# Napoliee/Expressive-FastSpeech2-Mandarin

Hardware: AMD Instinct MI355X
Metric: mel-frames/sec/GPU (batch-64 synth) at 1/2/4/8 MI355X; RTF (higher is better)
Workload: dtype bf16; 1 GPU; cfg2: batch=64 x 64 phonemes per GPU, ESD-Chinese-Singing-MFA model.yaml, FastSpeech2.forward eval bf16; global_batch=64, seq_len=64, mel_frames_per_gpu_batch=24883, T_max=430, parallelism=dp1 (independent shards, no collective), hip_graph=True

## Files before the change

### expressive-fastspeech2-mandarin_amd/csrc/ffn.hip

```cpp
#include <cstdlib>
#include <type_traits>
#include <utility>

#include "conv_common.h"
#include "fs2_common.h"

namespace {

#ifndef FFN_TRACE
#define FFN_TRACE 0
#endif
#ifndef FFN_ABLATE
#define FFN_ABLATE 0
#endif

constexpr int kD = 256;
constexpr int kChunk = 256;
constexpr int kUnit = 4096;
constexpr int kDepth = 4;

struct FfnArgs {
  ConvArgs e;
  const bf16 *w;
  const float *b1;
  uint32_t w_bytes;
  int nsplit;
  int ntiles;
  int *cnt;
  void *part;
  int acquire;
  int out_sc1;
  int prefetch;
  uint32_t part_bytes;
  const bf16 *wq;
  const float *bq;
  bf16 *qkv;
  int64_t qs;
  uint32_t wq_bytes;
  int nq;
  const bf16 *att;
  int64_t as;
  uint32_t att_bytes;
  const bf16 *wfc;
  const float *bfc, *g1, *be1;
  float eps1;
};

constexpr int part_bytes(int MB) { return 4 * 4 * MB * 64 * 16; }

constexpr int64_t ffn_weight_elems(int KS, int F) { return (int64_t)F * KS * kD + (int64_t)kD * F; }

__device__ __forceinline__ int xchunk(int r, int c) { return c ^ ((r & 3) << 1) ^ ((r & 4) ? 9 : 0); }

template <int N, typename Fn, int... I>
__device__ __forceinline__ void static_for_impl(Fn &&f, std::integer_sequence<int, I...>) {
  (f(std::integral_constant<int, I>{}), ...);
}
template <int N, typename Fn>
__device__ __forceinline__ void static_for(Fn &&f) {
  static_for_impl<N>(f, std::make_integer_sequence<int, N>{});
}

constexpr int kLgkm0 = 0xC07F;
constexpr int vm_imm(int n) { return (n & 15) | ((n >> 4) << 14) | 0x0F70; }

template <bool FUSED>
__device__ __forceinline__ float sumsq4(const f32x4 &d) {
#pragma clang fp contract(off)
  if constexpr (FUSED)
    return __builtin_fmaf(d[0], d[0], d[1] * d[1]) + __builtin_fmaf(d[2], d[2], d[3] * d[3]);
  else
    return (d[0] * d[0] + d[1] * d[1]) + (d[2] * d[2] + d[3] * d[3]);
}

template <int KS, int NCH, int MB, bool PRE = false, int NW = 4>
__global__ __launch_bounds__(NW * 64, NW / 4) void ffn_fused_kernel(FfnArgs p) {
  static_assert(NW == 4 || (NW == 8 && PRE && MB == 7 && KS == 9 && NCH == 4),
                "eight waves: the packed unsplit 112-row PRE launch only");
  constexpr int JB = 16 / NW;
  constexpr int NT = NW * 64;
  constexpr int BM = 16 * MB;
  constexpr uint32_t kPartBytes = (uint32_t)part_bytes(MB);
  constexpr int XROWS = BM + KS - 1;
  constexpr int XPITCH = 544;
  constexpr int XPIECES = (XROWS * XPITCH + 1023) / 1024;
  constexpr int XP_PER_WAVE = (XPIECES + NW - 1) / NW;
  constexpr int ZERO_OFF = 0;
  constexpr int X_OFF = 512;
  constexpr int H_OFF = X_OFF + NW * XP_PER_WAVE * 1024;
  constexpr int F = NCH * kChunk;
  constexpr int B1_OFF = H_OFF + BM * 512;
  constexpr int EP_OFF = B1_OFF + F * 4;
  constexpr int RED_OFF = EP_OFF + 3 * kD * 4;
  constexpr int ATT_OFF = H_OFF;
  constexpr int RED0_OFF = ATT_OFF + NW * XP_PER_WAVE * 1024;
  constexpr int SMEM0 = RED_OFF + BM * 16;
  constexpr int VEC0_OFF = RED0_OFF + 64 * 16;
  constexpr int SMEM1 = PRE && VEC0_OFF + 3 * kD * 4 > SMEM0 ? VEC0_OFF + 3 * kD * 4 : SMEM0;
  constexpr int XCH_OFF = SMEM1;
  constexpr int SMEM = SMEM1 + (NW == 8 ? 4 * 8 * 64 * 4 : 0);
  static_assert(SMEM <= 163840, "LDS");
  static_assert(MB <= 8, "pair-exchange slots");
  static_assert(BM * 528 <= NW * XP_PER_WAVE * 1024, "Q|K|V staging fits in the x region");
  constexpr int NK1 = KS * (kD / 32);
  constexpr int NK2 = kChunk / 32;
  constexpr int DEPTH = kDepth;
  static_assert(NK1 % DEPTH == 0 && NK2 % DEPTH == 0, "static register-ring slots");
  constexpr int SCR_OFF = SMEM + (FFN_TRACE ? 256 : 0);
  __shared__ __attribute__((aligned(16))) char smem[SCR_OFF + (PRE ? 0 : 4096)];

  const ConvArgs &a = p.e;
  const uint64_t t_entry = FFN_TRACE ? __builtin_readcyclecounter() : 0;
  const int tid = threadIdx.x, lane = tid & 63;
  const int wv = __builtin_amdgcn_readfirstlane(tid >> 6);
  const int w = NW == 8 ? wv >> 1 : wv;
  const int hf = NW == 8 ? wv & 1 : 0;
  const int col0 = wv * (16 * JB);
  const int M = a.rows_dev != nullptr ? min(*a.rows_dev, a.M) : a.M;
  const int S = p.nsplit;
  int tile = blockIdx.x, split = 0;
  if (S > 1) {
    const int ntiles = p.ntiles;
    const int L = (blockIdx.x & 7) * (gridDim.x >> 3) + (blockIdx.x >> 3);
    split = L / ntiles;
    tile = L - split * ntiles;
    if (split >= S) return;
  }
  const int m0 = tile * BM;
  if (m0 >= M) return;
  const int nchunks = NCH / S, c0 = split * nchunks, cend = c0 + nchunks;
  const int pad = a.pad, T = a.T;

  int vmask[MB];
  int padmask = 0;
  int2 rq[MB];
  int64_t rl[MB];
  if (NW == 8 || a.row_pos != nullptr) {
#pragma unroll
    for (int mb = 0; mb < MB; ++mb) rq[mb] = a.row_pos[min(m0 + mb * 16 + (lane & 15), M - 1)];
  } else {
#pragma unroll
    for (int mb = 0; mb < MB; ++mb) {
      const int m = min(m0 + mb * 16 + (lane & 15), M - 1);
      rq[mb] = make_int2(m % T, T);
    }
    if (a.lens != nullptr) {
#pragma unroll
      for (int mb = 0; mb < MB; ++mb) rl[mb] = a.lens[min(m0 + mb * 16 + (lane & 15), M - 1) / T];
    } else {
#pragma unroll
      for (int mb = 0; mb < MB; ++mb) rl[mb] = T;
    }
  }
#pragma unroll
  for (int mb = 0; mb < MB; ++mb) {
    const int m = m0 + mb * 16 + (lane & 15);
    int tpos = 0, tlen = 0;
    if (m < M) {
      tpos = rq[mb].x;
      tlen = rq[mb].y;
      if (NW == 4 && a.row_pos == nullptr && (int64_t)tpos >= rl[mb]) padmask |= 1 << mb;
    }
    int v = 0;
#pragma unroll
    for (int tap = 0; tap < KS; ++tap) v |= ((unsigned)(tpos + tap - pad) < (unsigned)tlen ? 1 : 0) << tap;
    vmask[mb] = v;
  }
  auto vec_dma = [&](const float *src, int piece, char *dst) {
    __builtin_amdgcn_raw_ptr_buffer_load_lds(make_rsrc(src, (uint32_t)(piece + 1) * 1024u),
                                             (__attribute__((address_space(3))) void *)dst, 16,
                                             (uint32_t)piece * 1024u + (uint32_t)lane * 16u, 0, 0, 0);
  };
  auto load_vectors = [&]() {
    for (int pc = wv; pc < F / 256; pc += NW) vec_dma(p.b1, pc, smem + B1_OFF + pc * 1024);
    if (wv < 3) vec_dma(wv == 0 ? a.bias : wv == 1 ? a.gamma : a.beta, 0, smem + EP_OFF + wv * 1024);
  };
  if constexpr (!PRE) load_vectors();
  if (tid < 32) *reinterpret_cast<float4 *>(smem + ZERO_OFF + 16 * tid) = make_float4(0.f, 0.f, 0.f, 0.f);
#pragma unroll
  for (int mb = 0; mb < MB; ++mb) asm volatile("" ::"v"(vmask[mb]));

  auto stamp = [&](int i) {
    if (FFN_TRACE) {
      __builtin_amdgcn_sched_barrier(0);
      const uint64_t t = __builtin_readcyclecounter();
      if (tid == 0) *reinterpret_cast<uint64_t *>(smem + SMEM + 8 * i) = t;
      __builtin_amdgcn_sched_barrier(0);
    }
  };
  auto pair_sum = [&](auto &pv, const auto &sv) {
    if constexpr (NW == 8) {
      constexpr int N = sizeof(pv) / sizeof(float);
      float *xp = reinterpret_cast<float *>(smem + XCH_OFF) + w * 512 + lane;
      if (hf == 0) {
#pragma unroll
        for (int i = 0; i < N; ++i) xp[i * 64] = pv[i];
      }
      __builtin_amdgcn_s_waitcnt(kLgkm0);
      __builtin_amdgcn_sched_barrier(0);
      __builtin_amdgcn_s_barrier();
      __builtin_amdgcn_sched_barrier(0);
      if (hf == 1) {
#pragma unroll
        for (int i = 0; i < N; ++i) pv[i] = (xp[i * 64] + sv[0][i]) + sv[1][i];
      }
    }
  };
  const rsrc_t wr = make_rsrc(p.w, p.w_bytes);
  auto tile_dma_range = [&](const void *src, uint32_t bytes, int64_t stride, int off, int i0, int i1) {
    const rsrc_t sr = make_rsrc(src, bytes);
    const uint32_t srow = (uint32_t)stride * 2u;
#pragma unroll
    for (int i = i0; i < i1; ++i) {
      const int pc = wv + NW * i;
      const int o = pc * 1024 + lane * 16;
      const int r = o / XPITCH, within = o - r * XPITCH;
      const int gm = m0 - pad + r;
      const bool ok = r < XROWS && within < 512 && gm >= 0 && gm < M;
      __builtin_amdgcn_raw_ptr_buffer_load_lds(
          sr, (__attribute__((address_space(3))) void *)(smem + off + pc * 1024), 16,
          ok ? (uint32_t)gm * srow + (uint32_t)within : kOOB, 0, 0, 0);
    }
  };
  auto tile_dma = [&](const void *src, uint32_t bytes, int64_t stride, int off) {
    tile_dma_range(src, bytes, stride, off, 0, XP_PER_WAVE);
  };
  constexpr uint32_t W2_BASE = (uint32_t)(F * KS * kD * 2);
  const uint32_t lane_off = (uint32_t)lane * 16u + (uint32_t)hf * 2048u;
  auto base1 = [&](int c) { return (uint32_t)((c * 4 + w) * NK1) * (uint32_t)kUnit; };
  auto base2 = [&](int c) { return W2_BASE + (uint32_t)(w * (F / 32) + c * NK2) * (uint32_t)kUnit; };
  bf16x8 pa[DEPTH][JB];
  auto load_at = [&](auto S, uint32_t so) {
    constexpr int s = decltype(S)::value;
    if (FFN_ABLATE & 2) return;
    __builtin_amdgcn_sched_barrier(0);
#pragma unroll
    for (int jb = 0; jb < JB; ++jb) {
      auto v = __builtin_amdgcn_raw_buffer_load_b128(wr, lane_off + jb * 1024, (FFN_ABLATE & 8) ? 0u : so, 0);
      pa[s][jb] = __builtin_bit_cast(bf16x8, v);
    }
    __builtin_amdgcn_sched_barrier(0);
  };
  auto ring_start = [&]() {
    static_for<DEPTH>([&](auto I) { load_at(I, base1(c0) + (uint32_t)(decltype(I)::value * kUnit)); });
  };
  if constexpr (!PRE) {
    if (S > 1 && p.prefetch) {
      const int nch = cend - c0;
      const int p1 = nch * 4 * NK1 * 4, p2q = nch * NK2 * 4;
      const uint32_t g1 = (uint32_t)(c0 * 4 * NK1) * (uint32_t)kUnit;
      constexpr uint32_t W2B = (uint32_t)(F * KS * kD * 2);
      const int per_xcd = (int)(gridDim.x >> 3);
      const int me = (int)(blockIdx.x >> 3) * 4 + w, nw = per_xcd * 4;
      for (int i = 0, pc = me; i < 16 && pc < p1 + 4 * p2q; ++i, pc += nw) {
        uint32_t off;
        if (pc < p1) {
          off = g1 + (uint32_t)pc * 1024u;
        } else {
          const int j = pc - p1, ww = j / p2q, r = j - ww * p2q;
          off = W2B + (uint32_t)(ww * (F / 32) + c0 * NK2) * (uint32_t)kUnit + (uint32_t)r * 1024u;
        }
        __builtin_amdgcn_raw_ptr_buffer_load_lds(wr, (__attribute__((address_space(3))) void *)(smem + SCR_OFF + w * 1024),
                                                 16, off + (uint32_t)lane * 16u, 0, 0, 0);
      }
    }
    tile_dma(a.x, a.x_bytes, a.xs, X_OFF);
    ring_start();
  } else {
    const int hr = lane & 15, hq = lane >> 4;
    if (wv < 3) vec_dma(wv == 0 ? p.bfc : wv == 1 ? p.g1 : p.be1, 0, smem + VEC0_OFF + wv * 1024);
    const rsrc_t fr = make_rsrc(p.wfc, (uint32_t)(kD * kD * 2));
    const uint32_t lane_o = lane_off;
    bf16x8 wf[8][JB];
#pragma unroll
    for (int ks = 0; ks < 8; ++ks)
#pragma unroll
      for (int jb = 0; jb < JB; ++jb)
        wf[ks][jb] = __builtin_bit_cast(bf16x8, __builtin_amdgcn_raw_buffer_load_b128(
                                                    fr, lane_o + (uint32_t)(jb * 1024), (uint32_t)((w * 8 + ks) * kUnit), 0));
    constexpr int PRE_SPLIT = (64 * XPITCH + 1023) / 1024 / NW + 1;
    static_assert(NW * PRE_SPLIT * 1024 >= 64 * XPITCH && PRE_SPLIT <= XP_PER_WAVE, "row pass 0 pieces");
    tile_dma_range(p.att, p.att_bytes, p.as, ATT_OFF, 0, PRE_SPLIT);
    tile_dma_range(a.x, a.x_bytes, a.xs, X_OFF, 0, PRE_SPLIT);
    tile_dma_range(p.att, p.att_bytes, p.as, ATT_OFF, PRE_SPLIT, XP_PER_WAVE);
    tile_dma_range(a.x, a.x_bytes, a.xs, X_OFF, PRE_SPLIT, XP_PER_WAVE);
    stamp(21);
    __builtin_amdgcn_s_waitcnt(vm_imm(2 * (XP_PER_WAVE - PRE_SPLIT)));
    __builtin_amdgcn_s_waitcnt(kLgkm0);
    __builtin_amdgcn_s_barrier();
    stamp(22);
    float *red0 = reinterpret_cast<float *>(smem + RED0_OFF);
    static_for<(XROWS + 63) / 64>([&](auto PS) {
      constexpr int ps = decltype(PS)::value;
      if constexpr (ps == 1) {
        asm volatile("s_waitcnt vmcnt(0)" ::: "memory");
        __builtin_amdgcn_s_barrier();
      }
      f32x4 a0[JB][4];
#pragma unroll
      for (int jb = 0; jb < JB; ++jb)
#pragma unroll
        for (int mb = 0; mb < 4; ++mb) a0[jb][mb] = f32x4{0.f, 0.f, 0.f, 0.f};
#pragma unroll
      for (int ks = 0; ks < 8; ++ks) {
        bf16x8 fb[4];
#pragma unroll
        for (int mb = 0; mb < 4; ++mb) {
          const int r = min(64 * ps + 16 * mb + hr, XROWS - 1);
          fb[mb] = *reinterpret_cast<const bf16x8 *>(smem + ATT_OFF + r * XPITCH + ks * 64 + hq * 16);
        }
#pragma unroll
        for (int mb = 0; mb < 4; ++mb)
#pragma unroll
          for (int jb = 0; jb < JB; ++jb)
            a0[jb][mb] = __builtin_amdgcn_mfma_f32_16x16x32_bf16(wf[ks][jb], fb[mb], a0[jb][mb], 0, 0, 0);
      }
      float part[4] = {0.f, 0.f, 0.f, 0.f}, mean[4], var[4];
      float sv[JB][4];
#pragma unroll
      for (int jb = 0; jb < JB; ++jb) {
        const int n = (NW == 8 ? col0 : w * 64) + jb * 16 + 4 * hq;
        const float4 bb = *reinterpret_cast<const float4 *>(smem + VEC0_OFF + 4 * n);
#pragma unroll
        for (int mb = 0; mb < 4; ++mb) {
          const int r = 64 * ps + 16 * mb + hr, gm = m0 - pad + r;
          const bool ok = r < XROWS && gm >= 0 && gm < M;
          bf16x4 xv = {(bf16)0.f, (bf16)0.f, (bf16)0.f, (bf16)0.f};
          if (ok) xv = *reinterpret_cast<const bf16x4 *>(smem + X_OFF + r * XPITCH + n * 2);
          f32x4 v = a0[jb][mb];
          v[0] = v[0] + bb.x + (float)xv[0];
          v[1] = v[1] + bb.y + (float)xv[1];
          v[2] = v[2] + bb.z + (float)xv[2];
          v[3] = v[3] + bb.w + (float)xv[3];
          a0[jb][mb] = v;
          if constexpr (NW == 8) {
            sv[jb][mb] = (v[0] + v[1]) + (v[2] + v[3]);
            part[mb] += sv[jb][mb];
          } else {
            part[mb] += (v[0] + v[1]) + (v[2] + v[3]);
          }
        }
      }
      auto reduce4 = [&](float (&pv)[4], float (&tot)[4]) {
        pair_sum(pv, sv);
        float t[4];
#pragma unroll
        for (int mb = 0; mb < 4; ++mb) t[mb] = __shfl_xor(pv[mb], 16, 64);
#pragma unroll
        for (int mb = 0; mb < 4; ++mb) pv[mb] += t[mb];
#pragma unroll
        for (int mb = 0; mb < 4; ++mb) t[mb] = __shfl_xor(pv[mb], 32, 64);
        if (NW == 4 || hf == 1) {
#pragma unroll
          for (int mb = 0; mb < 4; ++mb) red0[(mb * 16 + hr) * 4 + w] = pv[mb] + t[mb];
        }
        __builtin_amdgcn_s_waitcnt(kLgkm0);
        __builtin_amdgcn_s_barrier();
#pragma unroll
        for (int mb = 0; mb < 4; ++mb) {
          const float4 r4 = *reinterpret_cast<const float4 *>(red0 + (mb * 16 + hr) * 4);
          tot[mb] = (r4.x + r4.y) + (r4.z + r4.w);
        }
        __builtin_amdgcn_s_waitcnt(kLgkm0);
        __builtin_amdgcn_s_barrier();
      };
      reduce4(part, mean);
#pragma unroll
      for (int mb = 0; mb < 4; ++mb) {
        mean[mb] *= 1.0f / kD;
        float ss = 0.f;
#pragma unroll
        for (int jb = 0; jb < JB; ++jb) {
          f32x4 d = a0[jb][mb];
          d[0] -= mean[mb];
          d[1] -= mean[mb];
          d[2] -= mean[mb];
          d[3] -= mean[mb];
          a0[jb][mb] = d;
          if constexpr (NW == 8) {
            if constexpr (ps == 0)
              sv[jb][mb] = sumsq4<true>(d);
            else if (jb == 0 && mb < 3 && hf == 0)
              sv[jb][mb] = sumsq4<true>(d);
            else
              sv[jb][mb] = sumsq4<false>(d);
            ss += sv[jb][mb];
          } else {
            ss += (d[0] * d[0] + d[1] * d[1]) + (d[2] * d[2] + d[3] * d[3]);
          }
        }
        part[mb] = ss;
      }
      reduce4(part, var);
      float rstd[4], keep[4] = {1.f, 1.f, 1.f, 1.f};
#pragma unroll
      for (int mb = 0; mb < 4; ++mb) rstd[mb] = 1.0f / sqrtf(var[mb] * (1.0f / kD) + p.eps1);
      if (NW == 4 && a.lens != nullptr) {
#pragma unroll
        for (int mb = 0; mb < 4; ++mb) {
          const int gm = m0 - pad + 64 * ps + 16 * mb + hr;
          if (gm >= 0 && gm < M) {
            const int bb = gm / T;
            keep[mb] = (int64_t)(gm - bb * T) < a.lens[bb] ? 1.0f : 0.0f;
          }
        }
      }
#pragma unroll
      for (int jb = 0; jb < JB; ++jb) {
        const int n = (NW == 8 ? col0 : w * 64) + jb * 16 + 4 * hq;
        const float4 g = *reinterpret_cast<const float4 *>(smem + VEC0_OFF + 4 * (kD + n));
        const float4 be = *reinterpret_cast<const float4 *>(smem + VEC0_OFF + 4 * (2 * kD + n));
#pragma unroll
        for (int mb = 0; mb < 4; ++mb) {
          const int r = 64 * ps + 16 * mb + hr;
          const f32x4 d = a0[jb][mb];
          bf16x4 o;
          o[0] = (bf16)((d[0] * rstd[mb] * g.x + be.x) * keep[mb]);
          o[1] = (bf16)((d[1] * rstd[mb] * g.y + be.y) * keep[mb]);
          o[2] = (bf16)((d[2] * rstd[mb] * g.z + be.z) * keep[mb]);
          o[3] = (bf16)((d[3] * rstd[mb] * g.w + be.w) * keep[mb]);
          if (r < XROWS) *reinterpret_cast<bf16x4 *>(smem + X_OFF + r * XPITCH + n * 2) = o;
        }
      }
      stamp(23 + ps);
    });
    __builtin_amdgcn_s_waitcnt(kLgkm0);
    __builtin_amdgcn_s_barrier();
    load_vectors();
    ring_start();
  }


  const int hrow0 = lane & 15;
  const int hi = lane >> 4;
  bf16x8 f0[MB], f1[MB];
  auto bases_x = [&](int tap, int (&ad)[MB]) {
    const int base = X_OFF + (hrow0 + tap) * XPITCH + hi * 16;
#pragma unroll
    for (int mb = 0; mb < MB; ++mb) {
      const int keep = (FFN_ABLATE & 16) ? -1 : __builtin_amdgcn_sbfe(vmask[mb], tap, 1);
      ad[mb] = (base + mb * 16 * XPITCH) & keep;
    }
  };
  auto issue_x = [&](const int (&ad)[MB], auto KSI, bf16x8 (&f)[MB]) {
    if (FFN_ABLATE & 4) return;
    constexpr int off = decltype(KSI)::value * 64;
#pragma unroll
    for (int mb = 0; mb < MB; ++mb) f[mb] = *reinterpret_cast<const bf16x8 *>(smem + ad[mb] + off);
  };
  auto read_h = [&](int q, bf16x8 (&f)[MB]) {
    if (FFN_ABLATE & 4) return;
    const char *hp = smem + H_OFF + hrow0 * 512 + (xchunk(hrow0, 4 * q + hi) << 4);
#pragma unroll
    for (int mb = 0; mb < MB; ++mb) f[mb] = *reinterpret_cast<const bf16x8 *>(hp + mb * 8192);
  };

  f32x4 acc1[JB][MB], acc2[JB][MB];
#pragma unroll
  for (int i = 0; i < JB; ++i)
#pragma unroll
    for (int j = 0; j < MB; ++j) {
      acc1[i][j] = f32x4{0.f, 0.f, 0.f, 0.f};
      acc2[i][j] = f32x4{0.f, 0.f, 0.f, 0.f};
    }
  auto mma = [&](f32x4 (&acc)[JB][MB], const bf16x8 (&fa)[JB], const bf16x8 (&fb)[MB]) {
    if (FFN_ABLATE & 1) return;
#pragma unroll
    for (int mb = 0; mb < MB; ++mb)
#pragma unroll
      for (int jb = 0; jb < JB; ++jb)
        acc[jb][mb] = __builtin_amdgcn_mfma_f32_16x16x32_bf16(fa[jb], fb[mb], acc[jb][mb], 0, 0, 0);
  };
  auto bar = []() {
    __builtin_amdgcn_sched_barrier(0);
    __builtin_amdgcn_s_barrier();
    __builtin_amdgcn_sched_barrier(0);
  };
  auto trace_dump = [&](int last) {
    if (FFN_TRACE) {
      uint64_t *o = S > 1 ? reinterpret_cast<uint64_t *>(static_cast<char *>(p.part) + p.part_bytes + 256u * blockIdx.x)
                          : reinterpret_cast<uint64_t *>(static_cast<char *>(a.out) + (size_t)(a.M - 1 - blockIdx.x) * a.os * 2);
      for (int i = 0; i < 25; ++i) o[i] = *reinterpret_cast<const uint64_t *>(smem + SMEM + 8 * i);
      o[28] = t_entry;
      o[29] = (uint64_t)split;
      o[30] = (uint64_t)last;
      o[31] = (uint64_t)25;
    }
  };
  stamp(0);

  auto write_h = [&](int c) {
    float z;
    asm volatile("v_mov_b32 %0, 0" : "=v"(z));
#pragma unroll
    for (int jb = 0; jb < JB; ++jb) {
      const int j = (NW == 8 ? col0 : w * 64) + jb * 16 + 4 * hi;
      const float4 bb = *reinterpret_cast<const float4 *>(smem + B1_OFF + 4 * (c * kChunk + j));
#pragma unroll
      for (int mb = 0; mb < MB; ++mb) {
        const f32x4 v = acc1[jb][mb];
        bf16x4 o;
        o[0] = (bf16)fmaxf(v[0] + bb.x, 0.f);
        o[1] = (bf16)fmaxf(v[1] + bb.y, 0.f);
        o[2] = (bf16)fmaxf(v[2] + bb.z, 0.f);
        o[3] = (bf16)fmaxf(v[3] + bb.w, 0.f);
        const int m = hrow0 + mb * 16;
        *reinterpret_cast<bf16x4 *>(smem + H_OFF + m * 512 + (xchunk(m, j >> 3) << 4) + (j & 7) * 2) = o;
        acc1[jb][mb] = f32x4{z, z, z, z};
      }
    }
  };

  asm volatile("s_waitcnt vmcnt(%0)" ::"n"(JB * DEPTH) : "memory");
  __builtin_amdgcn_s_waitcnt(kLgkm0);
  bar();
  stamp(1);
  int bxc[MB], bxn[MB];
  bases_x(0, bxc);
  issue_x(bxc, std::integral_constant<int, 0>{}, f0);

  static_assert(DEPTH == 4 && kD / 32 == 8, "8 units per tap, 4-unit ring");
  auto unit1 = [&](auto KSI, int c, int tap) {
    constexpr int ks = decltype(KSI)::value, s = ks % DEPTH;
    if constexpr (ks + 1 < 8) {
      if constexpr (ks & 1)
        issue_x(bxc, std::integral_constant<int, ks + 1>{}, f0);
      else
        issue_x(bxc, std::integral_constant<int, ks + 1>{}, f1);
    } else {
      issue_x(bxn, std::integral_constant<int, 0>{}, f0);
    }
    if constexpr (ks & 1)
      mma(acc1, pa[s], f1);
    else
      mma(acc1, pa[s], f0);
    const uint32_t k1 = (uint32_t)(tap * 8 + ks + DEPTH) * (uint32_t)kUnit;
    if constexpr (ks + DEPTH < 8) {
      load_at(std::integral_constant<int, s>{}, base1(c) + k1);
    } else {
      const bool more = tap + 1 < KS;
      load_at(std::integral_constant<int, s>{},
              more ? base1(c) + k1 : base2(c) + (uint32_t)(((2 * w + ks - DEPTH) & (NK2 - 1)) * kUnit));
    }
  };
#pragma nounroll
  for (int c = c0; c < cend; ++c) {
#pragma nounroll
    for (int tap = 0; tap < KS; ++tap) {
      bases_x(tap + 1, bxn);
      static_for<8>([&](auto KSI) { unit1(KSI, c, tap); });
#pragma unroll
      for (int mb = 0; mb < MB; ++mb) bxc[mb] = bxn[mb];
    }
    stamp(2 + 2 * (c - c0));
    bar();
    write_h(c);
    __builtin_amdgcn_s_waitcnt(kLgkm0);
    stamp(3 + 2 * (c - c0));
    if constexpr (NW == 8) bar();
    read_h(2 * w, f0);
    const uint32_t next1 = c + 1 < cend ? base1(c + 1) : 0u;
    static_for<NK2>([&](auto Q) {
      constexpr int q = decltype(Q)::value;
      constexpr int s = q % DEPTH;
      if constexpr (q == 1 && NW == 4) {
        __builtin_amdgcn_s_waitcnt(kLgkm0);
        bar();
      }
      const int qn = (2 * w + q + 1) & (NK2 - 1);
      if constexpr (q + 1 == NK2) {
        bases_x(0, bxc);
        issue_x(bxc, std::integral_constant<int, 0>{}, f0);
      }
      else if constexpr (q & 1)
        read_h(qn, f0);
      else
        read_h(qn, f1);
      if constexpr (q & 1)
        mma(acc2, pa[s], f1);
      else
        mma(acc2, pa[s], f0);
      if constexpr (q + DEPTH < NK2)
        load_at(std::integral_constant<int, s>{}, base2(c) + (uint32_t)(((2 * w + q + DEPTH) & (NK2 - 1)) * kUnit));
      else
        load_at(std::integral_constant<int, s>{}, next1 + (uint32_t)((q + DEPTH - NK2) * kUnit));
    });
  }

  stamp(2 + 2 * NCH);
  asm volatile("s_waitcnt vmcnt(0)" ::: "memory");
  __builtin_amdgcn_s_waitcnt(kLgkm0);
  stamp(4 + 2 * NCH);
  if constexpr (NW == 4) {
    if (S > 1) {
      const rsrc_t pr = make_rsrc(p.part, p.part_bytes);
      auto pofs = [&](int sp, int nb, int mb) {
        return (uint32_t)(tile * S + sp) * (uint32_t)kPartBytes + (uint32_t)((((w * 4 + nb) * MB + mb) * 64 + lane) * 16);
      };
#pragma unroll
      for (int nb = 0; nb < 4; ++nb)
#pragma unroll
        for (int mb = 0; mb < MB; ++mb)
          __builtin_amdgcn_raw_buffer_store_b128(__builtin_bit_cast(__attribute__((ext_vector_type(4))) unsigned, acc2[nb][mb]),
                                                 pr, pofs(split, nb, mb), 0, 16);
      asm volatile("s_waitcnt vmcnt(0)" ::: "memory");
      __syncthreads();
      int *flag = reinterpret_cast<int *>(smem + RED_OFF);
      if (tid == 0) {
        const int old = __hip_atomic_fetch_add(p.cnt + tile, 1, __ATOMIC_RELAXED, __HIP_MEMORY_SCOPE_AGENT);
        const int last = old == S - 1;
        if (last) {
          __hip_atomic_store(p.cnt + tile, 0, __ATOMIC_RELAXED, __HIP_MEMORY_SCOPE_AGENT);
          if (p.acquire) __builtin_amdgcn_fence(__ATOMIC_ACQUIRE, "agent");
        }
        *flag = last;
      }
      asm volatile("s_waitcnt vmcnt(0)" ::: "memory");
      __syncthreads();
      stamp(19);
      if (FFN_TRACE && !*flag) {
        if (tid == 0) trace_dump(0);
      }
      if (!*flag) return;
      __syncthreads();
#pragma unroll
      for (int nb = 0; nb < 4; ++nb)
#pragma unroll
        for (int mb = 0; mb < MB; ++mb) acc1[nb][mb] = f32x4{0.f, 0.f, 0.f, 0.f};
      if constexpr (MB <= 4) {
        f32x4 v[3][4][MB];
        static_for<3>([&](auto J) {
          constexpr int j = decltype(J)::value;
          if (j < S - 1) {
            const int sp = j + (j >= split ? 1 : 0);
#pragma unroll
            for (int nb = 0; nb < 4; ++nb)
#pragma unroll
              for (int mb = 0; mb < MB; ++mb)
                v[j][nb][mb] = __builtin_bit_cast(f32x4, __builtin_amdgcn_raw_buffer_load_b128(pr, pofs(sp, nb, mb), 0, 16));
          }
        });
        static_for<4>([&](auto SP) {
          constexpr int sp = decltype(SP)::value;
          constexpr int jlo = sp < 3 ? sp : 2, jhi = sp > 0 ? sp - 1 : 0;
          if (sp < S) {
#pragma unroll
            for (int nb = 0; nb < 4; ++nb)
#pragma unroll
              for (int mb = 0; mb < MB; ++mb)
                acc1[nb][mb] += sp < split ? v[jlo][nb][mb] : (sp == split ? acc2[nb][mb] : v[jhi][nb][mb]);
          }
        });
      } else {
        for (int sp = 0; sp < S; ++sp) {
          if (sp == split) {
#pragma unroll
            for (int nb = 0; nb < 4; ++nb)
#pragma unroll
              for (int mb = 0; mb < MB; ++mb) acc1[nb][mb] += acc2[nb][mb];
          } else {
            f32x4 v[4][MB];
#pragma unroll
            for (int nb = 0; nb < 4; ++nb)
#pragma unroll
              for (int mb = 0; mb < MB; ++mb)
                v[nb][mb] = __builtin_bit_cast(f32x4, __builtin_amdgcn_raw_buffer_load_b128(pr, pofs(sp, nb, mb), 0, 16));
#pragma unroll
            for (int nb = 0; nb < 4; ++nb)
#pragma unroll
              for (int mb = 0; mb < MB; ++mb) acc1[nb][mb] += v[nb][mb];
          }
        }
      }
#pragma unroll
      for (int nb = 0; nb < 4; ++nb)
#pragma unroll
        for (int mb = 0; mb < MB; ++mb) acc2[nb][mb] = acc1[nb][mb];
      stamp(20);
    }
  }
  {
    int lane_e = lane;
    if constexpr (NW == 8) asm volatile("" : "+v"(lane_e));
    const int hrow0 = lane_e & 15, hi = lane_e >> 4;
    float *red = reinterpret_cast<float *>(smem + RED_OFF);
    const float inv_n = 1.0f / 256.0f;
    float4 b2v[JB], gv[JB], bev[JB];
#pragma unroll
    for (int nb = 0; nb < JB; ++nb) {
      const int n = (NW == 8 ? col0 : w * 64) + nb * 16 + 4 * hi;
      b2v[nb] = *reinterpret_cast<const float4 *>(smem + EP_OFF + 4 * n);
      gv[nb] = *reinterpret_cast<const float4 *>(smem + EP_OFF + 4 * (kD + n));
      bev[nb] = *reinterpret_cast<const float4 *>(smem + EP_OFF + 4 * (2 * kD + n));
    }
    float part[MB];
    float sv[JB][MB];
#pragma unroll
    for (int mb = 0; mb < MB; ++mb) {
      const int xr = mb * 16 + hrow0 + pad;
      float sum = 0.f;
#pragma unroll
      for (int nb = 0; nb < JB; ++nb) {
        const int n = (NW == 8 ? col0 : w * 64) + nb * 16 + 4 * hi;
        const bf16x4 xv = *reinterpret_cast<const bf16x4 *>(smem + X_OFF + xr * XPITCH + n * 2);
        f32x4 v = acc2[nb][mb];
        v[0] = v[0] + b2v[nb].x + (float)xv[0];
        v[1] = v[1] + b2v[nb].y + (float)xv[1];
        v[2] = v[2] + b2v[nb].z + (float)xv[2];
        v[3] = v[3] + b2v[nb].w + (float)xv[3];
        acc2[nb][mb] = v;
        if constexpr (NW == 8) {
          sv[nb][mb] = (v[0] + v[1]) + (v[2] + v[3]);
          sum += sv[nb][mb];
        } else {
          sum += (v[0] + v[1]) + (v[2] + v[3]);
        }
      }
      part[mb] = sum;
    }
    auto row_reduce = [&](float (&pv)[MB], float (&tot)[MB]) {
      pair_sum(pv, sv);
      float t[MB];
#pragma unroll
      for (int mb = 0; mb < MB; ++mb) t[mb] = __shfl_xor(pv[mb], 16, 64);
#pragma unroll
      for (int mb = 0; mb < MB; ++mb) pv[mb] += t[mb];
#pragma unroll
      for (int mb = 0; mb < MB; ++mb) t[mb] = __shfl_xor(pv[mb], 32, 64);
      if (NW == 4 || hf == 1) {
#pragma unroll
        for (int mb = 0; mb < MB; ++mb) red[(mb * 16 + hrow0) * 4 + w] = pv[mb] + t[mb];
      }
      __syncthreads();
#pragma unroll
      for (int mb = 0; mb < MB; ++mb) {
        const float4 r = *reinterpret_cast<const float4 *>(red + (mb * 16 + hrow0) * 4);
        tot[mb] = (r.x + r.y) + (r.z + r.w);
      }
      __syncthreads();
    };
    float mean[MB], var[MB];
    stamp(14);
    row_reduce(part, mean);
    stamp(15);
#pragma unroll
    for (int mb = 0; mb < MB; ++mb) {
      mean[mb] *= inv_n;
      float ss = 0.f;
#pragma unroll
      for (int nb = 0; nb < JB; ++nb) {
        f32x4 d = acc2[nb][mb];
        d[0] -= mean[mb];
        d[1] -= mean[mb];
        d[2] -= mean[mb];
        d[3] -= mean[mb];
        acc2[nb][mb] = d;
        if constexpr (NW == 8) {
          sv[nb][mb] = sumsq4<false>(d);
          ss += sv[nb][mb];
        } else {
          ss += (d[0] * d[0] + d[1] * d[1]) + (d[2] * d[2] + d[3] * d[3]);
        }
      }
      part[mb] = ss;
    }
    stamp(16);
    row_reduce(part, var);
    stamp(17);
    auto finish = [&](auto PADDED) {
      constexpr bool padded = decltype(PADDED)::value;
#pragma unroll
      for (int mb = 0; mb < MB; ++mb) {
        const float rstd = 1.0f / sqrtf(var[mb] * inv_n + a.eps);
        const int m = mb * 16 + hrow0;
        bool masked = false;
        int bb = 0;
        if constexpr (padded) {
          bb = (m0 + m) / T;
          masked = (padmask >> mb) & 1;
        }
#pragma unroll
        for (int nb = 0; nb < JB; ++nb) {
          const int n = (NW == 8 ? col0 : w * 64) + nb * 16 + 4 * hi;
          const f32x4 d = acc2[nb][mb];
          float y[4] = {d[0] * rstd * gv[nb].x + bev[nb].x, d[1] * rstd * gv[nb].y + bev[nb].y,
                        d[2] * rstd * gv[nb].z + bev[nb].z, d[3] * rstd * gv[nb].w + bev[nb].w};
          if constexpr (padded) {
            if (masked) y[0] = y[1] = y[2] = y[3] = 0.f;
            if (a.av1 != nullptr) {
              const float4 v1 = *reinterpret_cast<const float4 *>(a.av1 + (int64_t)bb * kD + n);
              y[0] += v1.x; y[1] += v1.y; y[2] += v1.z; y[3] += v1.w;
            }
            if (a.av2 != nullptr) {
              const float4 v2 = *reinterpret_cast<const float4 *>(a.av2 + (int64_t)bb * kD + n);
              y[0] += v2.x; y[1] += v2.y; y[2] += v2.z; y[3] += v2.w;
            }
          }
          bf16x4 o;
          o[0] = (bf16)y[0];
          o[1] = (bf16)y[1];
          o[2] = (bf16)y[2];
          o[3] = (bf16)y[3];
          *reinterpret_cast<bf16x4 *>(smem + H_OFF + m * 512 + (xchunk(m, n >> 3) << 4) + (n & 7) * 2) = o;
        }
      }
    };
    if (NW == 4 && (a.lens != nullptr || a.av1 != nullptr || a.av2 != nullptr))
      finish(std::true_type{});
    else
      finish(std::false_type{});
    __syncthreads();
    stamp(18);
    const uint32_t orow = (uint32_t)a.os * 2u;
    char *ob = static_cast<char *>(a.out);
#pragma unroll 2
    for (int i = tid; i < BM * 32; i += NT) {
      const int m = i >> 5, ch = i & 31;
      if (m0 + m < M) {
        const uint4 v = *reinterpret_cast<const uint4 *>(smem + H_OFF + m * 512 + (xchunk(m, ch) << 4));
        if (p.out_sc1)
          __builtin_amdgcn_raw_buffer_store_b128(__builtin_bit_cast(__attribute__((ext_vector_type(4))) unsigned, v),
                                                 make_rsrc(ob, 0x7fffffffu), (uint32_t)((m0 + m) * orow + ch * 16), 0, 16);
        else
          *reinterpret_cast<uint4 *>(ob + (size_t)(m0 + m) * orow + ch * 16) = v;
      }
    }
    if (p.wq != nullptr) {
      const rsrc_t qr = make_rsrc(p.wq, p.wq_bytes);
      auto qload = [&](auto S, uint32_t so) {
        constexpr int s = decltype(S)::value;
        __builtin_amdgcn_sched_barrier(0);
#pragma unroll
        for (int jb = 0; jb < JB; ++jb) {
          auto v = __builtin_amdgcn_raw_buffer_load_b128(qr, lane_off + jb * 1024, so, 0);
          pa[s][jb] = __builtin_bit_cast(bf16x8, v);
        }
        __builtin_amdgcn_sched_barrier(0);
      };
      constexpr int SPITCH = 528;
      const uint32_t qrow = (uint32_t)p.qs * 2u;
      char *qb = reinterpret_cast<char *>(p.qkv);
      const int npass = p.nq / 256;
      auto qbase = [&](int ps) { return (uint32_t)((ps * 4 + w) * 8) * (uint32_t)kUnit; };
      auto lbar = [&]() {
        __builtin_amdgcn_s_waitcnt(kLgkm0);
        __builtin_amdgcn_sched_barrier(0);
        __builtin_amdgcn_s_barrier();
        __builtin_amdgcn_sched_barrier(0);
      };
      static_for<DEPTH>([&](auto I) { qload(I, qbase(0) + (uint32_t)(decltype(I)::value * kUnit)); });
#pragma nounroll
      for (int ps = 0; ps < npass; ++ps) {
        const uint32_t base = qbase(ps);
        float z;
        asm volatile("v_mov_b32 %0, 0" : "=v"(z));
#pragma unroll
        for (int jb = 0; jb < JB; ++jb)
#pragma unroll
          for (int mb = 0; mb < MB; ++mb) acc1[jb][mb] = f32x4{z, z, z, z};
        read_h(0, f0);
        static_for<8>([&](auto Q) {
          constexpr int q = decltype(Q)::value, sl = q % DEPTH;
          if constexpr (q + 1 < 8) {
            if constexpr (q & 1)
              read_h(q + 1, f0);
            else
              read_h(q + 1, f1);
          }
          if constexpr (q & 1)
            mma(acc1, pa[sl], f1);
          else
            mma(acc1, pa[sl], f0);
          if constexpr (q + DEPTH < 8)
            qload(std::integral_constant<int, sl>{}, base + (uint32_t)((q + DEPTH) * kUnit));
          else
            qload(std::integral_constant<int, sl>{},
                  (ps + 1 < npass ? qbase(ps + 1) : qbase(0)) + (uint32_t)((q + DEPTH - 8) * kUnit));
        });
#pragma unroll
        for (int jb = 0; jb < JB; ++jb) {
          const int c = (NW == 8 ? col0 : w * 64) + jb * 16 + 4 * hi;
          const float4 bb = *reinterpret_cast<const float4 *>(p.bq + ps * 256 + c);
#pragma unroll
          for (int mb = 0; mb < MB; ++mb) {
            const f32x4 v = acc1[jb][mb];
            bf16x4 o;
            o[0] = (bf16)(v[0] + bb.x);
            o[1] = (bf16)(v[1] + bb.y);
            o[2] = (bf16)(v[2] + bb.z);
            o[3] = (bf16)(v[3] + bb.w);
            *reinterpret_cast<bf16x4 *>(smem + X_OFF + (hrow0 + mb * 16) * SPITCH + c * 2) = o;
          }
        }
        lbar();
#pragma unroll 2
        for (int i = tid; i < BM * 32; i += NT) {
          const int m = i >> 5, ch = i & 31;
          if (m0 + m < M) {
            const uint4 v = *reinterpret_cast<const uint4 *>(smem + X_OFF + m * SPITCH + ch * 16);
            if (p.out_sc1)
              __builtin_amdgcn_raw_buffer_store_b128(__builtin_bit_cast(__attribute__((ext_vector_type(4))) unsigned, v),
                                                     make_rsrc(qb, 0x7fffffffu),
                                                     (uint32_t)((m0 + m) * qrow + ps * 512 + ch * 16), 0, 16);
            else
              *reinterpret_cast<uint4 *>(qb + (size_t)(m0 + m) * qrow + ps * 512 + ch * 16) = v;
          }
        }
        lbar();
      }
      asm volatile("s_waitcnt vmcnt(0)" ::: "memory");
    }
  }
  stamp(5 + 2 * NCH);
  if (FFN_TRACE) {
    stamp(3 + 2 * NCH);
    __syncthreads();
    if (tid == 0) trace_dump(1);
  }
}

}

extern "C" int fs2_ffn(const fs2_ffn_desc *d, fs2_stream_t stream) {
  if (d == nullptr || d->x == nullptr || d->w == nullptr || d->b1 == nullptr || d->b2 == nullptr ||
      d->ln_gamma == nullptr || d->ln_beta == nullptr || d->out == nullptr)
    return FS2_EINVAL;
  if (d->B < 0 || d->T < 0 || d->x_row_stride < kD || (d->x_row_stride & 7) || d->out_row_stride < kD ||
      (d->out_row_stride & 7))
    return FS2_EINVAL;
  if (d->D != kD || !(d->F == 1024 || d->F == 512) || !(d->KS == 9 || d->KS == 3) || d->pad < 0 ||
      d->pad > d->KS - 1)
    return FS2_EUNSUPPORTED;
  if ((d->rows_dev == nullptr) != (d->row_pos == nullptr)) return FS2_EINVAL;
  if (d->rows_dev != nullptr && (d->lens != nullptr || d->addvec1 != nullptr || d->addvec2 != nullptr))
    return FS2_EINVAL;
  if (d->x == d->out) return FS2_EINVAL;
  const int S = d->nsplit <= 1 ? 1 : d->nsplit;
  if (!(S == 1 || S == 2 || S == 4) || S > d->F / kChunk) return FS2_EINVAL;
  const int64_t M64 = (int64_t)d->B * d->T;
  if (M64 > 0x7fffff00LL) return FS2_EINVAL;
  if (M64 == 0) return FS2_OK;
  const int64_t xb = M64 * d->x_row_stride * 2;
  const int64_t wb = ffn_weight_elems(d->KS, d->F) * 2;
  if (xb >= (1LL << 31)) return FS2_EUNSUPPORTED;

  FfnArgs p{};
  ConvArgs &a = p.e;
  a = ConvArgs{};
  a.x = d->x;
  a.xs = d->x_row_stride;
  a.w = d->w;
  a.bias = d->b2;
  a.B = d->B;
  a.T = d->T;
  a.Cin = kD;
  a.Cin_pad = kD;
  a.N = kD;
  a.KS = d->KS;
  a.pad = d->pad;
  a.M = (int)M64;
  a.epi = FS2_EPI_RES_LN;
  a.res = d->x;
  a.res_dt = FS2_BF16;
  a.rs = d->x_row_stride;
  a.gamma = d->ln_gamma;
  a.beta = d->ln_beta;
  a.eps = d->ln_eps;
  a.lens = d->lens;
  a.av1 = d->addvec1;
  a.av2 = d->addvec2;
  a.out = d->out;
  a.out_dt = FS2_BF16;
  a.os = d->out_row_stride;
  a.rows_dev = d->rows_dev;
  a.row_pos = reinterpret_cast<const int2 *>(d->row_pos);
  a.out_scale = 1.0f;
  a.ln_pairs = 1;
#ifdef FFN_EPI_DBG
  a.dbg = FFN_EPI_DBG;
#endif
  a.x_bytes = (uint32_t)xb;
  a.w_bytes = (uint32_t)wb;
  p.w = reinterpret_cast<const bf16 *>(d->w);
  p.b1 = d->b1;
  p.w_bytes = (uint32_t)wb;
  if (d->wqkv != nullptr) {
    if (d->bqkv == nullptr || d->qkv_out == nullptr || d->nqkv <= 0 || (d->nqkv % 256) ||
        d->qkv_row_stride < d->nqkv || (d->qkv_row_stride & 7) || d->qkv_out == d->x || d->qkv_out == d->out)
      return FS2_EINVAL;
    p.wq = reinterpret_cast<const bf16 *>(d->wqkv);
    p.bq = d->bqkv;
    p.qkv = reinterpret_cast<bf16 *>(d->qkv_out);
    p.qs = d->qkv_row_stride;
    p.nq = d->nqkv;
    p.wq_bytes = (uint32_t)((int64_t)d->nqkv * kD * 2);
  }
  const bool pre = d->pre_att != nullptr;
  if (pre) {
    if (d->pre_w == nullptr || d->pre_b == nullptr || d->pre_gamma == nullptr || d->pre_beta == nullptr ||
        d->pre_att_row_stride < kD || (d->pre_att_row_stride & 7) || d->pre_att == d->out)
      return FS2_EINVAL;
    const bool dec_form = d->rows_dev != nullptr;
    const bool enc_form = d->rows_dev == nullptr && d->tile_rows == 64;
    if (!(dec_form || enc_form) || d->KS != 9 || d->F != 1024) return FS2_EUNSUPPORTED;
    const int64_t ab = M64 * d->pre_att_row_stride * 2;
    if (ab >= (1LL << 31)) return FS2_EUNSUPPORTED;
    p.att = reinterpret_cast<const bf16 *>(d->pre_att);
    p.as = d->pre_att_row_stride;
    p.att_bytes = (uint32_t)ab;
    p.wfc = reinterpret_cast<const bf16 *>(d->pre_w);
    p.bfc = d->pre_b;
    p.g1 = d->pre_gamma;
    p.be1 = d->pre_beta;
    p.eps1 = d->pre_eps;
  }
  if (d->rows_max < 0 || !(d->tile_rows == 0 || d->tile_rows == 112 || d->tile_rows == 96 || d->tile_rows == 64))
    return FS2_EINVAL;
  const int MB = d->tile_rows == 64 ? 4 : d->tile_rows == 96 ? 6 : 7, BM = 16 * MB;
  if (MB == 6 && (d->KS != 9 || d->F != 1024)) return FS2_EUNSUPPORTED;
  const int64_t kPartBytes = part_bytes(MB);
  const int64_t Mg = (d->rows_dev != nullptr && d->rows_max > 0 && d->rows_max < M64) ? d->rows_max : M64;
  a.M = (int)Mg;
  const int ntiles = (int)((Mg + BM - 1) / BM);
  int nwg = ntiles;
  p.nsplit = S;
  p.ntiles = ntiles;
  static const int acquire = [] {
    const char *e = getenv("FS2_FFN_ACQUIRE");
    return (e != nullptr && e[0] == '1') ? 1 : 0;
  }();
  p.acquire = acquire;
  static const int out_sc1 = [] {
    const char *e = getenv("FS2_OUT_SC1");
    return (e != nullptr && e[0] == '0') ? 0 : 1;
  }();
  p.out_sc1 = out_sc1;
  static const int ffn_prefetch = [] {
    const char *e = getenv("FS2_FFN_PREFETCH");
    return (e != nullptr && e[0] == '1') ? 1 : 0;
  }();
  p.prefetch = ffn_prefetch;
  auto ffn_w8 = [] {
    const char *e = getenv("FS2_FFN_W8");
    return !(e != nullptr && e[0] == '0');
  };
  if (S > 1) {
    if (d->splitk_ws == nullptr || ntiles > 1024 ||
        d->splitk_ws_bytes < 4096 + (int64_t)ntiles * S * kPartBytes + (FFN_TRACE ? 256LL * (ntiles * S + 8) : 0) ||
        (int64_t)ntiles * S * kPartBytes >= (1LL << 31))
      return FS2_EINVAL;
    p.cnt = static_cast<int *>(d->splitk_ws);
    p.part = static_cast<char *>(d->splitk_ws) + 4096;
    p.part_bytes = (uint32_t)((int64_t)ntiles * S * kPartBytes);
    nwg = (ntiles * S + 7) & ~7;
  }
  const int nch = d->F / kChunk;
  hipStream_t s = as_stream(stream);
  auto run = [&](void (*kernel)(FfnArgs), int nw) { hipLaunchKernelGGL(kernel, dim3(nwg), dim3(nw * 64), 0, s, p); };
  auto go = [&](auto KSC, auto NCHC, auto PREC) {
    constexpr int ks = decltype(KSC)::value, nc = decltype(NCHC)::value;
    constexpr bool pr = decltype(PREC)::value;
    if (MB == 4) return run(ffn_fused_kernel<ks, nc, 4, pr>, 4);
    if constexpr (ks == 9 && nc == 4)
      if (MB == 6) return run(ffn_fused_kernel<9, 4, 6, pr>, 4);
    if constexpr (pr)
      if (S == 1 && d->rows_dev != nullptr && ffn_w8()) return run(ffn_fused_kernel<9, 4, 7, true, 8>, 8);
    run(ffn_fused_kernel<ks, nc, 7, pr>, 4);
  };
  using I9 = std::integral_constant<int, 9>;
  using I3 = std::integral_constant<int, 3>;
  using C4 = std::integral_constant<int, 4>;
  using C2 = std::integral_constant<int, 2>;
  if (pre)
    go(I9{}, C4{}, std::true_type{});
  else if (d->KS == 9 && nch == 4)
    go(I9{}, C4{}, std::false_type{});
  else if (d->KS == 9 && nch == 2)
    go(I9{}, C2{}, std::false_type{});
  else if (d->KS == 3 && nch == 4)
    go(I3{}, C4{}, std::false_type{});
  else if (d->KS == 3 && nch == 2)
    go(I3{}, C2{}, std::false_type{});
  else
    return FS2_EUNSUPPORTED;
  FS2_CHECK_LAUNCH();
  return FS2_OK;
}

extern "C" int64_t fs2_ffn_weight_elems(int KS, int F) { return ffn_weight_elems(KS, F); }
```

Measured before the change: 18.09 million mel-frames/s.

## Split FFN prologue attention-projection rows across wave halves for 8-wave blocks

Adds a dedicated 8-wave prologue path: each wave pair now splits the 128 rows between its two halves instead of splitting columns, so every wave computes a 64-column by 64-row slab. This removes the cross-half pair exchange through LDS and the two row passes. The fc weights are streamed through a 4-slot register ring rather than held fully in registers, which lowers register pressure. The tap-mask computation is deferred until after the DMAs are issued so it overlaps with the loads. The reduction scratch area is doubled to give the mean and variance passes separate buffers, which also drops one barrier.

New measurement: 18.24 million mel-frames/s (median of 6 runs). No clear change (+0.8%).

```diff
diff --git a/expressive-fastspeech2-mandarin_amd/csrc/ffn.hip b/expressive-fastspeech2-mandarin_amd/csrc/ffn.hip
--- a/expressive-fastspeech2-mandarin_amd/csrc/ffn.hip
+++ b/expressive-fastspeech2-mandarin_amd/csrc/ffn.hip
@@ -95,7 +95,8 @@
   constexpr int ATT_OFF = H_OFF;
   constexpr int RED0_OFF = ATT_OFF + NW * XP_PER_WAVE * 1024;
   constexpr int SMEM0 = RED_OFF + BM * 16;
-  constexpr int VEC0_OFF = RED0_OFF + 64 * 16;
+  constexpr int RED0_BYTES = NW == 8 ? 2 * 128 * 16 : 64 * 16;
+  constexpr int VEC0_OFF = RED0_OFF + RED0_BYTES;
   constexpr int SMEM1 = PRE && VEC0_OFF + 3 * kD * 4 > SMEM0 ? VEC0_OFF + 3 * kD * 4 : SMEM0;
   constexpr int XCH_OFF = SMEM1;
   constexpr int SMEM = SMEM1 + (NW == 8 ? 4 * 8 * 64 * 4 : 0);
@@ -152,19 +153,21 @@
       for (int mb = 0; mb < MB; ++mb) rl[mb] = T;
     }
   }
-#pragma unroll
-  for (int mb = 0; mb < MB; ++mb) {
-    const int m = m0 + mb * 16 + (lane & 15);
-    int tpos = 0, tlen = 0;
-    if (m < M) {
-      tpos = rq[mb].x;
-      tlen = rq[mb].y;
-      if (NW == 4 && a.row_pos == nullptr && (int64_t)tpos >= rl[mb]) padmask |= 1 << mb;
-    }
-    int v = 0;
-#pragma unroll
-    for (int tap = 0; tap < KS; ++tap) v |= ((unsigned)(tpos + tap - pad) < (unsigned)tlen ? 1 : 0) << tap;
-    vmask[mb] = v;
+  if constexpr (NW == 4) {
+#pragma unroll
+    for (int mb = 0; mb < MB; ++mb) {
+      const int m = m0 + mb * 16 + (lane & 15);
+      int tpos = 0, tlen = 0;
+      if (m < M) {
+        tpos = rq[mb].x;
+        tlen = rq[mb].y;
+        if (a.row_pos == nullptr && (int64_t)tpos >= rl[mb]) padmask |= 1 << mb;
+      }
+      int v = 0;
+#pragma unroll
+      for (int tap = 0; tap < KS; ++tap) v |= ((unsigned)(tpos + tap - pad) < (unsigned)tlen ? 1 : 0) << tap;
+      vmask[mb] = v;
+    }
   }
   auto vec_dma = [&](const float *src, int piece, char *dst) {
     __builtin_amdgcn_raw_ptr_buffer_load_lds(make_rsrc(src, (uint32_t)(piece + 1) * 1024u),
@@ -177,8 +180,10 @@
   };
   if constexpr (!PRE) load_vectors();
   if (tid < 32) *reinterpret_cast<float4 *>(smem + ZERO_OFF + 16 * tid) = make_float4(0.f, 0.f, 0.f, 0.f);
-#pragma unroll
-  for (int mb = 0; mb < MB; ++mb) asm volatile("" ::"v"(vmask[mb]));
+  if constexpr (NW == 4) {
+#pragma unroll
+    for (int mb = 0; mb < MB; ++mb) asm volatile("" ::"v"(vmask[mb]));
+  }
 
   auto stamp = [&](int i) {
     if (FFN_TRACE) {
@@ -265,6 +270,149 @@
       }
     }
     tile_dma(a.x, a.x_bytes, a.xs, X_OFF);
+    ring_start();
+  } else if constexpr (NW == 8) {
+    const int hr = lane & 15, hq = lane >> 4;
+    if (wv < 3) vec_dma(wv == 0 ? p.bfc : wv == 1 ? p.g1 : p.be1, 0, smem + VEC0_OFF + wv * 1024);
+    const rsrc_t fr = make_rsrc(p.wfc, (uint32_t)(kD * kD * 2));
+    constexpr int FD = 4;
+    bf16x8 wf[FD][4];
+    auto load_fc = [&](auto S, int ks) {
+      constexpr int s = decltype(S)::value;
+      __builtin_amdgcn_sched_barrier(0);
+#pragma unroll
+      for (int jb = 0; jb < 4; ++jb)
+        wf[s][jb] = __builtin_bit_cast(bf16x8, __builtin_amdgcn_raw_buffer_load_b128(
+                                                   fr, (uint32_t)lane * 16u + (uint32_t)(jb * 1024), (uint32_t)((w * 8 + ks) * kUnit), 0));
+      __builtin_amdgcn_sched_barrier(0);
+    };
+    static_for<FD>([&](auto I) { load_fc(I, decltype(I)::value); });
+    tile_dma(p.att, p.att_bytes, p.as, ATT_OFF);
+    tile_dma(a.x, a.x_bytes, a.xs, X_OFF);
+    static_assert(4 * FD + 2 * XP_PER_WAVE < 64, "vmcnt is six bits");
+    __builtin_amdgcn_sched_barrier(0);
+    __builtin_amdgcn_s_waitcnt(vm_imm(4 * FD + 2 * XP_PER_WAVE));
+    __builtin_amdgcn_sched_barrier(0);
+#pragma unroll
+    for (int mb = 0; mb < MB; ++mb) {
+      const bool in = m0 + mb * 16 + (lane & 15) < M;
+      const int tpos = in ? rq[mb].x : 0, tlen = in ? rq[mb].y : 0;
+      int v = 0;
+#pragma unroll
+      for (int tap = 0; tap < KS; ++tap) v |= ((unsigned)(tpos + tap - pad) < (unsigned)tlen ? 1 : 0) << tap;
+      vmask[mb] = v;
+    }
+#pragma unroll
+    for (int mb = 0; mb < MB; ++mb) asm volatile("" ::"v"(vmask[mb]));
+    stamp(21);
+    asm volatile("s_waitcnt vmcnt(0)" ::: "memory");
+    __builtin_amdgcn_s_waitcnt(kLgkm0);
+    __builtin_amdgcn_s_barrier();
+    stamp(22);
+    const int r0 = 64 * hf + hr;
+    f32x4 a0[4][4];
+#pragma unroll
+    for (int jb = 0; jb < 4; ++jb)
+#pragma unroll
+      for (int mb = 0; mb < 4; ++mb) a0[jb][mb] = f32x4{0.f, 0.f, 0.f, 0.f};
+    static_for<8>([&](auto KSI) {
+      constexpr int ks = decltype(KSI)::value, s = ks % FD;
+      bf16x8 fb[4];
+#pragma unroll
+      for (int mb = 0; mb < 4; ++mb) {
+        const int r = min(r0 + 16 * mb, XROWS - 1);
+        fb[mb] = *reinterpret_cast<const bf16x8 *>(smem + ATT_OFF + r * XPITCH + ks * 64 + hq * 16);
+      }
+#pragma unroll
+      for (int mb = 0; mb < 4; ++mb)
+#pragma unroll
+        for (int jb = 0; jb < 4; ++jb)
+          a0[jb][mb] = __builtin_amdgcn_mfma_f32_16x16x32_bf16(wf[s][jb], fb[mb], a0[jb][mb], 0, 0, 0);
+      if constexpr (ks + FD < 8) load_fc(std::integral_constant<int, s>{}, ks + FD);
+    });
+    stamp(23);
+    float part[4] = {0.f, 0.f, 0.f, 0.f}, mean[4], var[4];
+#pragma unroll
+    for (int jb = 0; jb < 4; ++jb) {
+      const int n = w * 64 + jb * 16 + 4 * hq;
+      const float4 bb = *reinterpret_cast<const float4 *>(smem + VEC0_OFF + 4 * n);
+#pragma unroll
+      for (int mb = 0; mb < 4; ++mb) {
+        const int r = r0 + 16 * mb, gm = m0 - pad + r;
+        const bool ok = r < XROWS && gm >= 0 && gm < M;
+        bf16x4 xv = {(bf16)0.f, (bf16)0.f, (bf16)0.f, (bf16)0.f};
+        if (ok) xv = *reinterpret_cast<const bf16x4 *>(smem + X_OFF + r * XPITCH + n * 2);
+        f32x4 v = a0[jb][mb];
+        v[0] = v[0] + bb.x + (float)xv[0];
+        v[1] = v[1] + bb.y + (float)xv[1];
+        v[2] = v[2] + bb.z + (float)xv[2];
+        v[3] = v[3] + bb.w + (float)xv[3];
+        a0[jb][mb] = v;
+        part[mb] += (v[0] + v[1]) + (v[2] + v[3]);
+      }
+    }
+    auto reduce4 = [&](float (&pv)[4], float (&tot)[4], float *rd) {
+      float t[4];
+#pragma unroll
+      for (int mb = 0; mb < 4; ++mb) t[mb] = __shfl_xor(pv[mb], 16, 64);
+#pragma unroll
+      for (int mb = 0; mb < 4; ++mb) pv[mb] += t[mb];
+#pragma unroll
+      for (int mb = 0; mb < 4; ++mb) t[mb] = __shfl_xor(pv[mb], 32, 64);
+#pragma unroll
+      for (int mb = 0; mb < 4; ++mb) rd[(r0 + 16 * mb) * 4 + w] = pv[mb] + t[mb];
+      __builtin_amdgcn_s_waitcnt(kLgkm0);
+      __builtin_amdgcn_s_barrier();
+#pragma unroll
+      for (int mb = 0; mb < 4; ++mb) {
+        const float4 r4 = *reinterpret_cast<const float4 *>(rd + (r0 + 16 * mb) * 4);
+        tot[mb] = (r4.x + r4.y) + (r4.z + r4.w);
+      }
+    };
+    float *red0 = reinterpret_cast<float *>(smem + RED0_OFF);
+    reduce4(part, mean, red0);
+#pragma unroll
+    for (int mb = 0; mb < 4; ++mb) {
+      mean[mb] *= 1.0f / kD;
+      float ss = 0.f;
+#pragma unroll
+      for (int jb = 0; jb < 4; ++jb) {
+        f32x4 d = a0[jb][mb];
+        d[0] -= mean[mb];
+        d[1] -= mean[mb];
+        d[2] -= mean[mb];
+        d[3] -= mean[mb];
+        a0[jb][mb] = d;
+        if (jb == 0 && mb < 3)
+          ss += sumsq4<true>(d);
+        else
+          ss += hf == 0 ? sumsq4<true>(d) : sumsq4<false>(d);
+      }
+      part[mb] = ss;
+    }
+    reduce4(part, var, red0 + 128 * 4);
+    float rstd[4];
+#pragma unroll
+    for (int mb = 0; mb < 4; ++mb) rstd[mb] = 1.0f / sqrtf(var[mb] * (1.0f / kD) + p.eps1);
+#pragma unroll
+    for (int jb = 0; jb < 4; ++jb) {
+      const int n = w * 64 + jb * 16 + 4 * hq;
+      const float4 g = *reinterpret_cast<const float4 *>(smem + VEC0_OFF + 4 * (kD + n));
+      const float4 be = *reinterpret_cast<const float4 *>(smem + VEC0_OFF + 4 * (2 * kD + n));
+#pragma unroll
+      for (int mb = 0; mb < 4; ++mb) {
+        const int r = r0 + 16 * mb;
+        const f32x4 d = a0[jb][mb];
+        bf16x4 o;
+        o[0] = (bf16)(d[0] * rstd[mb] * g.x + be.x);
+        o[1] = (bf16)(d[1] * rstd[mb] * g.y + be.y);
+        o[2] = (bf16)(d[2] * rstd[mb] * g.z + be.z);
+        o[3] = (bf16)(d[3] * rstd[mb] * g.w + be.w);
+        if (r < XROWS) *reinterpret_cast<bf16x4 *>(smem + X_OFF + r * XPITCH + n * 2) = o;
+      }
+    }
+    stamp(24);
+    load_vectors();
     ring_start();
   } else {
     const int hr = lane & 15, hq = lane >> 4;
@@ -316,10 +464,9 @@
             a0[jb][mb] = __builtin_amdgcn_mfma_f32_16x16x32_bf16(wf[ks][jb], fb[mb], a0[jb][mb], 0, 0, 0);
       }
       float part[4] = {0.f, 0.f, 0.f, 0.f}, mean[4], var[4];
-      float sv[JB][4];
 #pragma unroll
       for (int jb = 0; jb < JB; ++jb) {
-        const int n = (NW == 8 ? col0 : w * 64) + jb * 16 + 4 * hq;
+        const int n = w * 64 + jb * 16 + 4 * hq;
         const float4 bb = *reinterpret_cast<const float4 *>(smem + VEC0_OFF + 4 * n);
 #pragma unroll
         for (int mb = 0; mb < 4; ++mb) {
@@ -333,16 +480,10 @@
           v[2] = v[2] + bb.z + (float)xv[2];
           v[3] = v[3] + bb.w + (float)xv[3];
           a0[jb][mb] = v;
-          if constexpr (NW == 8) {
-            sv[jb][mb] = (v[0] + v[1]) + (v[2] + v[3]);
-            part[mb] += sv[jb][mb];
-          } else {
-            part[mb] += (v[0] + v[1]) + (v[2] + v[3]);
-          }
+          part[mb] += (v[0] + v[1]) + (v[2] + v[3]);
         }
       }
       auto reduce4 = [&](float (&pv)[4], float (&tot)[4]) {
-        pair_sum(pv, sv);
         float t[4];
 #pragma unroll
         for (int mb = 0; mb < 4; ++mb) t[mb] = __shfl_xor(pv[mb], 16, 64);
@@ -350,10 +491,8 @@
         for (int mb = 0; mb < 4; ++mb) pv[mb] += t[mb];
 #pragma unroll
         for (int mb = 0; mb < 4; ++mb) t[mb] = __shfl_xor(pv[mb], 32, 64);
-        if (NW == 4 || hf == 1) {
-#pragma unroll
-          for (int mb = 0; mb < 4; ++mb) red0[(mb * 16 + hr) * 4 + w] = pv[mb] + t[mb];
-        }
+#pragma unroll
+        for (int mb = 0; mb < 4; ++mb) red0[(mb * 16 + hr) * 4 + w] = pv[mb] + t[mb];
         __builtin_amdgcn_s_waitcnt(kLgkm0);
         __builtin_amdgcn_s_barrier();
 #pragma unroll
@@ -377,17 +516,7 @@
           d[2] -= mean[mb];
           d[3] -= mean[mb];
           a0[jb][mb] = d;
-          if constexpr (NW == 8) {
-            if constexpr (ps == 0)
-              sv[jb][mb] = sumsq4<true>(d);
-            else if (jb == 0 && mb < 3 && hf == 0)
-              sv[jb][mb] = sumsq4<true>(d);
-            else
-              sv[jb][mb] = sumsq4<false>(d);
-            ss += sv[jb][mb];
-          } else {
-            ss += (d[0] * d[0] + d[1] * d[1]) + (d[2] * d[2] + d[3] * d[3]);
-          }
+          ss += (d[0] * d[0] + d[1] * d[1]) + (d[2] * d[2] + d[3] * d[3]);
         }
         part[mb] = ss;
       }
@@ -395,7 +524,7 @@
       float rstd[4], keep[4] = {1.f, 1.f, 1.f, 1.f};
 #pragma unroll
       for (int mb = 0; mb < 4; ++mb) rstd[mb] = 1.0f / sqrtf(var[mb] * (1.0f / kD) + p.eps1);
-      if (NW == 4 && a.lens != nullptr) {
+      if (a.lens != nullptr) {
 #pragma unroll
         for (int mb = 0; mb < 4; ++mb) {
           const int gm = m0 - pad + 64 * ps + 16 * mb + hr;
@@ -407,8 +536,8 @@
       }
 #pragma unroll
       for (int jb = 0; jb < JB; ++jb) {
-        const int n = (NW == 8 ? col0 : w * 64) + jb * 16 + 4 * hq;
-        const float4 g = *reinterpret_cast<const float4 *>(smem + VEC0_OFF + 4 * (kD + n));
+        const int n = w * 64 + jb * 16 + 4 * hq;
+        const float4 g =*reinterpret_cast<const float4 *>(smem + VEC0_OFF + 4 * (kD + n));
         const float4 be = *reinterpret_cast<const float4 *>(smem + VEC0_OFF + 4 * (2 * kD + n));
 #pragma unroll
         for (int mb = 0; mb < 4; ++mb) {
```
